# THUwangcy/ReChorus

Hardware: AMD Instinct MI355X
Metric: ranked (1+K)-tuples/sec (higher is better)
Workload: dtype f32; 1 GPU; BPRMF fit step: emb_size=64, num_neg=99, 10000001-item / 1000001-user tables, Zipf(1.0) users+positives, uniform negatives, B=65536 tuples/GPU/step, optimizer=SGD (row-wise, l2=0), int64 ids, fp32; batch_per_gpu=65536, num_neg=99, emb_size=64, n_items=10000001, optimizer=SGD, parallelism=single GPU

## Files before the change

include/rechorus_hip.h:

```cpp
#ifndef RECHORUS_HIP_H
#define RECHORUS_HIP_H

#include <stddef.h>
#include <stdint.h>

#ifdef __cplusplus
extern "C" {
#endif

typedef void* rc_stream_t;

enum rc_status {
  RC_OK = 0,
  RC_ERR_INVALID_ARG = -1,
  RC_ERR_WORKSPACE = -2,
  RC_ERR_HIP = -3,
  RC_ERR_UNSUPPORTED = -4
};

enum rc_opt {
  RC_OPT_SGD = 0,
  RC_OPT_ADAM = 1,
  RC_OPT_ADAGRAD = 2,
  RC_OPT_ADADELTA = 3
// ... 339 lines not shown
size_t rc_bucket_bitmap_bytes(int64_t range_a);
int rc_bucket_multi_bitmap(const int64_t* ids_a, int64_t n_a, int64_t range_a, uint32_t* bitmap, void* ws,
                           size_t ws_bytes, rc_stream_t stream);

size_t rc_plan_update_workspace_bytes(int64_t n_occ, int d);
int rc_plan_update(float* W, float* m, float* v, int d, const rc_plan_row* rows, const uint32_t* n_rows,
                   const uint32_t* occ, int64_t n_occ, const float* coef, const float* src, const int64_t* src_index,
                   int div, const float* src2, int64_t n_split, const rc_opt_hyper* h, void* ws, size_t ws_bytes,
                   rc_stream_t stream);

int rc_plan_update_pair(float* W_a, float* m_a, float* v_a, float* W_b, float* m_b, float* v_b, int d,
                        const rc_plan_row* rows, const uint32_t* n_rows, const uint32_t* occ, int64_t n_occ,
                        const float* src_a, const float* src_b, int64_t src_ld, int64_t occ_base, const rc_opt_hyper* h,
                        uint32_t* counters, void* ws, size_t ws_bytes, rc_stream_t stream);

int rc_plan_row_sums(float* out, int d, const rc_plan_row* rows, const uint32_t* n_rows, const uint32_t* occ,
                     int64_t n_occ, const float* coef, const float* src, const int64_t* src_index, int div,
                     const float* src2, int64_t n_split, void* ws, size_t ws_bytes, rc_stream_t stream);

int rc_plan_distinct(const rc_plan_row* rows, const uint32_t* n_rows, const uint32_t* occ, int64_t occ_base,
                     int64_t n_list, int64_t* uniq, int64_t* inverse, rc_stream_t stream);

size_t rc_bprmf_step_workspace_bytes(int B, int C, int d);

int rc_bprmf_step_pipeline(int mode);

int rc_bprmf_train_step(float* U, float* I, float* mU, float* vU, float* mI, float* vI,
                        const int64_t* uid, const int64_t* iid, int B, int C, int d,
                        int64_t n_users, int64_t n_items, const rc_opt_hyper* h,
                        float inv_b, float* loss_out, float* pred, void* ws,
                        size_t ws_bytes, rc_stream_t stream, float* phase_ms);

typedef struct rc_step_ticket {
  uint64_t generation;
  uint64_t ws;
  int32_t slot;
  int32_t device;
  int32_t B, C, d;
  int32_t flavour;
  int64_t n_users, n_items;
  uint64_t reserved[2];
} rc_step_ticket;

int rc_bprmf_train_step_ahead(float* U, float* I, float* mU, float* vU, float* mI, float* vI,
                              const int64_t* uid, const int64_t* iid, uint64_t generation,
                              const int64_t* next_uid, const int64_t* next_iid, uint64_t next_generation,
// ... 259 lines not shown
```

rechorus_amd/_lib.py:

```python
import ctypes as C
import os

_PKG = os.path.dirname(os.path.abspath(__file__))
LIB_PATH = os.environ.get("RC_LIB_PATH") or os.path.join(_PKG, "librechorus_hip.so")

RC_OK = 0
RC_OPT_SGD, RC_OPT_ADAM, RC_OPT_ADAGRAD, RC_OPT_ADADELTA = 0, 1, 2, 3
RC_SEG_SKIP_SINGLETONS = 1
OPT_BY_NAME = {"SGD": RC_OPT_SGD, "Adam": RC_OPT_ADAM, "Adagrad": RC_OPT_ADAGRAD, "Adadelta": RC_OPT_ADADELTA}


class RechorusHipMissing(ImportError):
    pass


class RechorusHipError(RuntimeError):
    def __init__(self, fn, code, text):
        super().__init__(f"{fn} failed (rc_status {code}): {text}")
        self.code = code


class OptHyper(C.Structure):
    _fields_ = [
        ("opt", C.c_int),
# ... 164 lines not shown
    "rc_neumf_head_fwd_bwd": (_i, [_p, _p, _i64, _p, _p, _i64, _p, _p, _p, _p, _p, _i, _i, _i, _i, _f, _p, _p, _p, _p, _i64, _p, _p, _i64,
                                   _p, _p, _p, _p, _sz, _p]),
    "rc_bench_mix": (_i, [_p, _i, _p, _i64, _f, _i, _p, C.POINTER(C.c_float), _p]),
    "rc_bench_mfma": (_i, [_i, _p, C.POINTER(C.c_float), _p]),
    "rc_linear_fwd": (_i, [_p, _p, _p, _i64, _i, _i, _i, _f, _p, C.c_uint32, _p, _p, _sz, _p]),
    "rc_linear_fwd_workspace_bytes": (_sz, [_i64, _i, _i]),
    "rc_linear_bwd_workspace_bytes": (_sz, [_i64, _i, _i]),
    "rc_linear_bwd": (_i, [_p, _p, _p, _p, _i64, _i, _i, _f, _i, _f, _p, _p, _p, _p, _sz, _p]),
    "rc_tower_tail_supported": (_i, [_i64, _i, _i]),
    "rc_tower_tail_workspace_bytes": (_sz, [_i64, _i, _i]),
    "rc_tower_tail_fwd": (_i, [_p, _p, _p, _p, _p, _i64, _i, _i, _f, _p, C.c_uint32, _p, _p, _p]),
    "rc_tower_tail_bwd": (_i, [_p, _p, _p, _p, _p, _i64, _i, _i, _f, _i, _f, _p, _p, _p, _p, _p, _p, _sz, _p]),
    "rc_bucket_plan_supported": (_i, [_i64, _i64, _i64, _i64]),
    "rc_bucket_plan_workspace_bytes": (_sz, [_i64, _i64]),
    "rc_bucket_plan_flags_bytes": (_sz, [_i64]),
    "rc_bucket_plan_status_ptr": (_p, [_p, _i64, _i64]),
    "rc_bucket_plan": (_i, [_p, _i64, _i64, _p, _i64, _i64, _i, _p, _p, _p, _p, _p, _p, _p, _sz, _p]),
    "rc_plan_update_workspace_bytes": (_sz, [_i64, _i]),
    "rc_plan_update": (_i, [_p, _p, _p, _i, _p, _p, _p, _i64, _p, _p, _p, _i, _p, _i64, _hp, _p, _sz, _p]),
    "rc_plan_update_pair": (_i, [_p, _p, _p, _p, _p, _p, _i, _p, _p, _p, _i64, _p, _p, _i64, _i64, _hp, _p, _p, _sz, _p]),
    "rc_plan_row_sums": (_i, [_p, _i, _p, _p, _p, _i64, _p, _p, _p, _i, _p, _i64, _p, _sz, _p]),
    "rc_plan_distinct": (_i, [_p, _p, _p, _i64, _i64, _p, _p, _p]),
    "rc_bprmf_step_workspace_bytes": (_sz, [_i, _i, _i]),
    "rc_bprmf_step_pipeline": (_i, [_i]),
    "rc_bprmf_train_step": (_i, [_p, _p, _p, _p, _p, _p, _p, _p, _i, _i, _i, _i64, _i64, _hp, _f,
                                 _p, _p, _p, _sz, _p, C.POINTER(C.c_float)]),
    "rc_bprmf_step_ahead_reset": (_i, [_tp, _p]),
    "rc_bprmf_train_step_ahead": (_i, [_p, _p, _p, _p, _p, _p, _p, _p, _u64, _p, _p, _u64, _tp, _i, _i, _i, _i64, _i64, _hp, _f,
                                       _p, _p, _p, _sz, _p, C.POINTER(C.c_float)]),
    "rc_bucket_bitmap_bytes": (_sz, [_i64]),
    "rc_bucket_multi_bitmap": (_i, [_p, _i64, _i64, _p, _p, _sz, _p]),
    "rc_lgcn_check_shape": (_i, [_i, _i, _i64, _i64]),
    "rc_lgcn_propagate_fwd": (_i, [_gp, _p, _p, _i, _i, _p, _p, _p, _p, _p]),
    "rc_lgcn_propagate_bwd": (_i, [_gp, _p, _p, _i, _i, _p, _p, _p, _p, _p, _p]),
    "rc_directau_check_shape": (_i, [_i, _i64]),
    "rc_directau_workspace_bytes": (_sz, [_i, _i64]),
    "rc_directau_fwd": (_i, [_p, _p, _p, _p, _i64, _i, _f, _i, _p, _sz, _p, _p, _p]),
    "rc_directau_bwd": (_i, [_p, _i64, _i, _f, _f, _f, _p, _sz, _p, _p, _p]),
    "rc_buir_check_shape": (_i, [_i, _i64]),
    "rc_buir_workspace_bytes": (_sz, [_i, _i64]),
    "rc_buir_fwd": (_i, [_p] * 8 + [_i64, _i, _p, _sz, _p, _p, _p]),
    "rc_buir_bwd": (_i, [_p] * 9 + [_i64, _i, _p, _sz, _p, _p, _p, _p, _p]),
    "rc_buir_query": (_i, [_p, _p, _p, _p, _i64, _i, _p, _p, _p]),
    "rc_buir_scores": (_i, [_p, _p, _p, _p, _i64, _i64, _i, _p, _p]),
    "rc_buir_ema": (_i, [_p, _p, _i64, _p, _p, _i64, _dbl, _p]),
    "rc_comirec_check_shape": (_i, [_i, _i, _i, _i]),
# ... 107 lines not shown
```

rechorus_amd/csrc/bprmf_fused.hip:

```cpp
#include "bprmf_step.hpp"
#include "fused_body.hpp"
#include "small_plan.hpp"

namespace rc {

template <int D, int GS, int CPL, int MODE>
__global__ __launch_bounds__(kBlock, (fused_min_waves<CPL, MODE>())) void bprmf_fwd_bwd_kernel(
    const float* __restrict__ U, const float* I,
    const int64_t* __restrict__ uid, const int64_t* __restrict__ iid, int B, int C,
    float inv_b, float* __restrict__ pred, float* __restrict__ loss_vec,
    float* __restrict__ gpred, float* __restrict__ ugrad, FusedUpd upd) {
  bprmf_fwd_bwd_body<D, GS, CPL, MODE, kBlock>(U, I, uid, iid, B, C, inv_b, pred, loss_vec, gpred, ugrad, upd,
                                               (int64_t)blockIdx.x, nullptr);
}

template <int D, int GS, int CPL>
__global__ __launch_bounds__(kSmallThreads) void small_front_kernel(
    const float* __restrict__ U, const float* I, const int64_t* __restrict__ uid, const int64_t* __restrict__ iid,
    int B, int C, float inv_b, float* __restrict__ pred, float* __restrict__ loss_vec, float* __restrict__ gpred,
    float* __restrict__ ugrad, float* __restrict__ ub, SmallPlanArgs plan) {
  extern __shared__ __attribute__((aligned(16))) unsigned char small_smem[];
  if (blockIdx.x < (unsigned)kSmallPlanWgs) {
    small_plan_block(plan, blockIdx.x, small_smem);
    return;
  }
  FusedUpd none;
  none.I = nullptr; none.M = nullptr; none.V = nullptr; none.single = nullptr;
  bprmf_fwd_bwd_body<D, GS, CPL, MODE_NONE, kSmallThreads>(U, I, uid, iid, B, C, inv_b, pred, loss_vec, gpred, ugrad, none,
                                                           (int64_t)blockIdx.x - kSmallPlanWgs, ub);
}

constexpr int kGenericMaxC = 4096;
constexpr int kGenericMaxDChunks = 8;

__global__ __launch_bounds__(kBlock) void bprmf_fwd_bwd_generic_kernel(
    const float* __restrict__ U, const float* __restrict__ I,
    const int64_t* __restrict__ uid, const int64_t* __restrict__ iid, int B, int C, int d,
    float inv_b, float* __restrict__ pred, float* __restrict__ loss_vec,
    float* __restrict__ gpred, float* __restrict__ ugrad) {
  extern __shared__ float smem[];
  const int lane = threadIdx.x & 63;
  const int wib = threadIdx.x >> 6;
  const int64_t t_raw = (int64_t)blockIdx.x * (kBlock / 64) + wib;
  const bool tv = t_raw < B;
  const int64_t t = tv ? t_raw : (int64_t)B - 1;
  float* sp = smem + (size_t)wib * C;
  const float* ur = U + uid[t] * d;
  const int64_t* ids = iid + t * C;
  for (int c = 0; c < C; ++c) {
    const float* ir = I + ids[c] * d;
// ... 61 lines not shown
  const float* U;
  const float* I;
  const int64_t* uid;
  const int64_t* iid;
  int B, C;
  float inv_b;
  float* pred;
  float* loss_vec;
  float* gpred;
  float* ugrad;
  int mode;
  const char* who;
  FusedUpd upd;
  hipStream_t s;
  const SmallPlanArgs* small;
  float* ub;
};

template <int D, int GS, int CPL>
static int launch_fused(const FusedCall& f) {
  constexpr int TPW = 64 / ((D / 4) * GS);
  constexpr int TPB = TPW * (kBlock / 64);
  const int blocks = (f.B + TPB - 1) / TPB;
  if (f.small) {
    constexpr int TPB_S = TPW * (kSmallThreads / 64);
    const int fblocks = (f.B + TPB_S - 1) / TPB_S;
    auto kern = small_front_kernel<D, GS, CPL>;
    static bool attr_done = false;
    if (!attr_done) {
      RC_HIP(hipFuncSetAttribute(reinterpret_cast<const void*>(kern), hipFuncAttributeMaxDynamicSharedMemorySize, (int)kSmallLdsBytes));
      attr_done = true;
    }
    hipLaunchKernelGGL(kern, dim3(kSmallPlanWgs + fblocks), dim3(kSmallThreads), kSmallLdsBytes, f.s, f.U, f.I, f.uid, f.iid,
                       f.B, f.C, f.inv_b, f.pred, f.loss_vec, f.gpred, f.ugrad, f.ub, *f.small);
    RC_LAUNCH_CHECK();
    return RC_OK;
  }
  return dispatch_or_fail<MODE_NONE, MODE_SGD, MODE_ADAM, MODE_ADAGRAD>(f.who, "update mode", f.mode, [&](auto M) -> int {
    hipLaunchKernelGGL((bprmf_fwd_bwd_kernel<D, GS, CPL, M()>), dim3(blocks), dim3(kBlock), 0, f.s, f.U, f.I, f.uid, f.iid, f.B, f.C,
                       f.inv_b, f.pred, f.loss_vec, f.gpred, f.ugrad, f.upd);
    RC_LAUNCH_CHECK();
    return RC_OK;
  });
}

template <int D>
// ... 53 lines not shown
  hipStream_t s = as_stream(stream);
  if (aligned16(U, I, ugrad) && register_path_ok(d, C)) {
    FusedCall f;
    memset(&f, 0, sizeof(f));
    f.U = U; f.I = I; f.uid = uid; f.iid = iid; f.B = B; f.C = C; f.inv_b = inv_b;
    f.pred = pred; f.loss_vec = loss_vec; f.gpred = gpred; f.ugrad = ugrad;
    f.mode = MODE_NONE; f.s = s; f.who = "rc_bprmf_fwd_bwd";
    bool handled = false;
    const int rc_ = run_fused(f, d, &handled);
    if (handled) return rc_;
  }
  if (C > kGenericMaxC || d > 64 * kGenericMaxDChunks)
    return fail(RC_ERR_UNSUPPORTED,
                "rc_bprmf_fwd_bwd: no kernel for C=%d d=%d (generic path: C<=%d, d<=%d)", C, d,
                kGenericMaxC, 64 * kGenericMaxDChunks);
  const int blocks = (B + (kBlock / 64) - 1) / (kBlock / 64);
  const size_t shmem = (size_t)(kBlock / 64) * C * sizeof(float);
  hipLaunchKernelGGL(bprmf_fwd_bwd_generic_kernel, dim3(blocks), dim3(kBlock), shmem, s, U, I,
                     uid, iid, B, C, d, inv_b, pred, loss_vec, gpred, ugrad);
  RC_LAUNCH_CHECK();
  return RC_OK;
}

extern "C" int rc_bprmf_fwd_bwd_update(const float* U, float* I, float* mI, float* vI, const int64_t* uid,
                                       const int64_t* iid, const uint8_t* single, const uint32_t* multi, int B, int C, int d,
                                       float inv_b, const rc_opt_hyper* h, float* pred, float* loss_vec, float* gpred, float* ugrad,
                                       rc_stream_t stream) {
  static const char* who = "rc_bprmf_fwd_bwd_update";
  if (B == 0) return RC_OK;
  RC_REQUIRE((single != nullptr) != (multi != nullptr), "%s: exactly one of single / multi must be given", who);
  RC_REQUIRE(U && I && uid && iid && h && loss_vec && gpred && ugrad, "%s: null pointer", who);
  RC_REQUIRE(B > 0 && C >= 2 && d >= 1, "%s: bad shape B=%d C=%d d=%d", who, B, C, d);
  if (!register_path_ok(d, C))
    return fail(RC_ERR_UNSUPPORTED,
                "%s: no register-resident kernel for d=%d C=%d "
                "(check rc_bprmf_fused_supported; use rc_bprmf_fwd_bwd + rc_segmented_update)", who, d, C);
  FusedCall f;
  memset(&f, 0, sizeof(f));
  RC_TRY(fill_opt_scalars(who, h, &f.upd.o));
  f.mode = mode_of(h);
  RC_TRY(opt_state_check(who, f.mode, mI != nullptr, vI != nullptr));
  RC_REQUIRE(aligned16(U, I, ugrad, mI, vI), "%s: tables must be 16-byte aligned", who);
  f.U = U; f.I = I; f.uid = uid; f.iid = iid; f.B = B; f.C = C; f.inv_b = inv_b;
  f.pred = pred; f.loss_vec = loss_vec; f.gpred = gpred; f.ugrad = ugrad;
  f.upd.I = I; f.upd.M = mI; f.upd.V = vI; f.upd.single = single; f.upd.multi = multi;
  f.s = as_stream(stream); f.who = who;
  bool handled = false;
  const int rc_ = run_fused(f, d, &handled);
  if (!handled) return fail(RC_ERR_UNSUPPORTED, "%s: dispatch failed", who);
  return rc_;
}

namespace rc {
int small_front_launch(const BprmfStep& st, float* ub, const SmallPlanArgs& plan) {
  const int d = st.d, C = st.C;
  RC_REQUIRE(aligned16(st.U, st.I, st.ugrad, ub) && register_path_ok(d, C),
             "small-batch step: unsupported shape or alignment (d=%d C=%d)", d, C);
  FusedCall f;
  memset(&f, 0, sizeof(f));
  f.U = st.U; f.I = st.I; f.uid = st.uid; f.iid = st.iid; f.B = st.B; f.C = C; f.inv_b = st.inv_b;
  f.pred = st.pred; f.loss_vec = st.loss_vec; f.gpred = st.gpred; f.ugrad = st.ugrad;
  f.mode = MODE_NONE; f.s = st.s; f.small = &plan; f.ub = ub; f.who = "rc_bprmf_train_step";
  bool handled = false;
  const int rc_ = run_fused(f, d, &handled);
  if (!handled) return fail(RC_ERR_UNSUPPORTED, "small-batch step: dispatch failed (d=%d C=%d)", d, C);
  return rc_;
}
}
```

rechorus_amd/csrc/bprmf_step.hpp:

```cpp
#pragma once
#include "common.hpp"
#include "opt_math.hpp"
#include "plan.hpp"

namespace rc {

struct SmallPlanArgs;

struct BprmfStep {
  float *U, *I;
  float *mU, *vU, *mI, *vI;
  const int64_t* uid;
  const int64_t* iid;
  int B, C, d;
  int64_t n_users, n_items;
  const rc_opt_hyper* h;
  OptScalars o;
  int mode;
  float inv_b;
  float* loss_out;
  float* pred;
  float *gpred, *ugrad, *loss_vec;
  hipStream_t s;
  int64_t n_i() const { return (int64_t)B * C; }
};

bool small_step_supported(int64_t n_i, int64_t B, int64_t n_items, int64_t n_users, int d);
size_t small_step_extra_bytes(int64_t n, int64_t B, int d);
int small_step_launch(const BprmfStep& st, void* extra, hipEvent_t* ev_mid);
int small_front_launch(const BprmfStep& st, float* ub, const SmallPlanArgs& plan);

int plan_bprmf_step_updates(const BprmfStep& st, const rc_plan_row* rows_i, const uint32_t* n_rows_i, const rc_plan_row* rows_u,
                            const uint32_t* n_rows_u, const uint32_t* occ, uint32_t* counters, const PlanLongWs& lw,
                            const PlanMedList& med, hipEvent_t* ev_items_done);

}
```

rechorus_amd/csrc/common.hpp:

```cpp
#pragma once
#include <cstdarg>
#include <cstdint>
#include <cstdio>
#include <cstring>
#include <cmath>
#include <type_traits>

#include <hip/hip_runtime.h>

#include "../../include/rechorus_hip.h"

namespace rc {

char* last_error_buf();

inline int fail(int code, const char* fmt, ...) {
  va_list ap;
  va_start(ap, fmt);
  vsnprintf(last_error_buf(), 512, fmt, ap);
  va_end(ap);
  return code;
}

#define RC_REQUIRE(cond, ...)                                   \
// ... 33 lines not shown

template <int... Vs, class F>
inline int dispatch_or_fail(const char* who, const char* what, int v, F&& f) {
  int rc = RC_OK;
  if (dispatch_int<Vs...>(v, &rc, f)) return rc;
  return fail(RC_ERR_UNSUPPORTED, "%s: %s %d has no kernel", who, what, v);
}

struct Carver {
  char* base;
  size_t off = 0;
  explicit Carver(void* p) : base(reinterpret_cast<char*>(p)) {}
  template <typename T>
  T* take(size_t count) {
    T* p = reinterpret_cast<T*>(base + off);
    off += align_up(count * sizeof(T), 256);
    return p;
  }
};

constexpr int kWave = 64;
constexpr int kBlock = 256;
constexpr int kMaxGridX = 1 << 30;

int device_cus();

#if defined(__HIPCC__)

template <int CTRL>
__device__ __forceinline__ float dpp_mov(float x) {
  int xi = __float_as_int(x);
  int r = __builtin_amdgcn_update_dpp(xi, xi, CTRL, 0xF, 0xF, false);
  return __int_as_float(r);
}

template <int NT, bool STAGED>
__device__ __forceinline__ float fixed_order_partial(const float* __restrict__ x, int64_t n, int tid) {
  float acc = 0.f;
  int64_t done = 0;
  if (reinterpret_cast<uintptr_t>(x) % 16 == 0) {
    const int64_t n4 = n / 4;
    const float4* x4 = reinterpret_cast<const float4*>(x);
    if (!STAGED || n4 <= (int64_t)4 * NT) {
#pragma unroll 8
      for (int64_t i = tid; i < n4; i += NT) {
        const float4 v = x4[i];
// ... 73 lines not shown
```

rechorus_amd/csrc/fused_body.hpp:

```cpp
#pragma once
#include "bpr_math.hpp"
#include "common.hpp"
#include "opt_math.hpp"

namespace rc {

struct FusedUpd {
  float* I;
  float* M;
  float* V;
  const uint8_t* single;
  const uint32_t* multi;
  OptScalars o;
};

template <int S>
__device__ __forceinline__ float tuple_allreduce_sum(float x) {
  x = row_allreduce_sum<(S < 16 ? S : 16)>(x);
  if (S >= 32) x += __shfl_xor(x, 16, 64);
  if (S >= 64) x += __shfl_xor(x, 32, 64);
  return x;
}
template <int S>
__device__ __forceinline__ float tuple_allreduce_max(float x) {
  if (S >= 2) x = fmaxf(x, dpp_mov<0xB1>(x));
  if (S >= 4) x = fmaxf(x, dpp_mov<0x4E>(x));
  if (S >= 8) x = fmaxf(x, dpp_mov<0x141>(x));
  if (S >= 16) x = fmaxf(x, dpp_mov<0x140>(x));
  if (S >= 32) x = fmaxf(x, __shfl_xor(x, 16, 64));
  if (S >= 64) x = fmaxf(x, __shfl_xor(x, 32, 64));
  return x;
}

template <int CPL_, int MODE_>
constexpr int fused_min_waves() {
  return (MODE_ == MODE_ADAM || MODE_ == MODE_ADAGRAD) ? (CPL_ >= 20 ? 2 : 3) : (CPL_ >= 26 ? 2 : (CPL_ >= 20 ? 3 : 4));
}
template <int D, int GS, int CPL>
struct FusedGeom {
  static constexpr int LPR = D / 4;
  static constexpr int S = LPR * GS;
  static_assert(S <= 64 && (64 % S) == 0, "tuple must fit a wave");
  static constexpr int TPW = 64 / S;
  static constexpr int SLOTS = GS * CPL;
  static constexpr int NPL = (SLOTS + S - 1) / S;
  static constexpr bool COAL = S == 64 && SLOTS <= 128;
  static constexpr int ID_SLOTS = COAL ? SLOTS : 1;
};

struct TupleIds {
  int64_t u;
  int64_t ia, ib;
};

template <int D, int GS, int CPL>
__device__ __forceinline__ TupleIds fused_load_ids(const int64_t* __restrict__ uid, const int64_t* __restrict__ iid, int64_t t,
                                                   int C, int lane) {
  using G = FusedGeom<D, GS, CPL>;
  TupleIds k;
  k.u = uid[t];
  k.ia = k.ib = 0;
  if (G::COAL) {
    const int64_t* ids = iid + t * C;
    const int c0 = lane, c1 = lane + 64;
    k.ia = ids[c0 < C ? c0 : 0];
    if (G::SLOTS > 64) k.ib = ids[c1 < C ? c1 : 0];
  }
  return k;
}

// ... 155 lines not shown
    if (cc[k] < 0) g = 0.f;
    if (s < SLOTS) strip[s] = g;
    if (tv && cc[k] >= 0) {
      gpred[t * C + cc[k]] = g;
      if (pred != nullptr) pred[t * C + cc[k]] = pc[k];
    }
  }
  __builtin_amdgcn_fence(__ATOMIC_RELEASE, "wavefront");
  __builtin_amdgcn_wave_barrier();
  __builtin_amdgcn_fence(__ATOMIC_ACQUIRE, "wavefront");

  float4 acc = make_float4(0.f, 0.f, 0.f, 0.f);
  float gs[CPL];
#pragma unroll
  for (int j = 0; j < CPL; ++j) {
    const float g = strip[grp * CPL + j];
    acc.x = fmaf(g, r[j].x, acc.x);
    acc.y = fmaf(g, r[j].y, acc.y);
    acc.z = fmaf(g, r[j].z, acc.z);
    acc.w = fmaf(g, r[j].w, acc.w);
    if (MODE == MODE_ADAM || MODE == MODE_ADAGRAD) gs[j] = g;
  }
  if (MODE == MODE_SGD) {
#pragma unroll
    for (int j = 0; j < CPL; ++j) {
      if (smask & (1u << j)) {
        const int64_t id = ids[j * GS + grp];
        const float g = strip[grp * CPL + j];
        const float4 gi = make_float4(g * u4.x, g * u4.y, g * u4.z, g * u4.w);
        opt_row4_group<MODE, LPR>(upd.o, upd.I, upd.M, upd.V, (size_t)id * LPR + l, r[j], gi);
      }
    }
  }
  acc.x = groups_allreduce_sum<LPR, S>(acc.x);
  acc.y = groups_allreduce_sum<LPR, S>(acc.y);
  acc.z = groups_allreduce_sum<LPR, S>(acc.z);
  acc.w = groups_allreduce_sum<LPR, S>(acc.w);
  if (tv && grp == 0) reinterpret_cast<float4*>(ugrad + t * D)[l] = acc;

  if (MODE == MODE_ADAM || MODE == MODE_ADAGRAD) {
    constexpr int GRP = 5;
#pragma unroll
    for (int j0 = 0; j0 < CPL; j0 += GRP) {
      float4 mm[GRP], vv[GRP];
      size_t idx[GRP];
#pragma unroll
      for (int q = 0; q < GRP; ++q) {
        const int j = j0 + q;
        mm[q] = vv[q] = make_float4(0.f, 0.f, 0.f, 0.f);
        idx[q] = 0;
        if (j < CPL && ((smask >> j) & 1u)) {
          idx[q] = (size_t)ids[j * GS + grp] * LPR + l;
          mm[q] = load_stream4(reinterpret_cast<const float4*>(upd.M) + idx[q]);
// ... 48 lines not shown
```

rechorus_amd/csrc/plan.hpp:

```cpp
#pragma once
#include "common.hpp"
#include "opt_math.hpp"

namespace rc {

constexpr int kPlanTile = 8192;
constexpr int kPlanThreads = 512;
constexpr int kPlanWaves = kPlanThreads / 64;
constexpr int kPlanRounds = kPlanTile / kPlanThreads;
constexpr int kPlanMaxBuckets = 4096;
constexpr int kPlanMaxShift = 13;
constexpr int kPlanMinShift = 8;
constexpr int kPlanLongSeg = 32;
constexpr int kPlanChunk = 256;
constexpr int kPlanIdxOcc = 4;
constexpr int kPlanBodyOcc = 2;

struct PlanGeom {
  int ok;
  int shift;
  uint32_t nb_a, nb_b, nb;
  uint32_t base_b;
  uint32_t tiles;
  int bucket_bits;
// ... 58 lines not shown
  int emit_long;
  PlanMedList med;
  int bitmap_in_bucket;
  PlanLongWs lw;
};
int plan_launch(const PlanArgs& a, hipStream_t s, hipEvent_t* ev_after_scatter);
int plan_launch_front(const PlanArgs& a, bool bitmap, hipStream_t s);
constexpr size_t kPlanBitmapWords = (size_t)kPlanMaxBuckets << (kPlanMaxShift - 5);
int plan_launch_back(const PlanArgs& a, hipStream_t s);
int plan_prepare();

struct PlanTable { float* W; float* M; float* V; };

struct PlanGrad {
  const float* coef;
  const float* src;
  const int64_t* src_index;
  int div;
  const float* src2;
  uint32_t n_split;
  const float* src2b;
  int pair;
  uint32_t pair_ld4;
};

}
```

rechorus_amd/csrc/plan_update.hip:

```cpp
#include "bprmf_step.hpp"
#include "plan.hpp"

namespace rc {

constexpr bool LPR_OK(int D) { return D / 4 <= 64 && 64 % (D / 4) == 0; }

struct PlanSide {
  PlanTable t;
  PlanTable tb;
  PlanGrad g;
  const rc_plan_row* rows;
  const uint32_t* n_rows;
};

struct PlanUpdArgs {
  PlanSide side[2];
  const uint32_t* occ;
  uint32_t* counters;
  PlanLongWs lw;
  OptScalars o;
  const float* loss_vec;
  int64_t loss_n;
  float loss_scale;
  float* loss_out;
// ... 103 lines not shown
#pragma unroll
    for (int h = 0; h < H; ++h) {
      if (g0 + h >= nr) break;
      if (!act[h]) {
        if (plan_long) plan_long_row<LPR>(a, e[h], side, l);
        continue;
      }
      if (e[h].n > 1) padd4(acc[h], s1[h]);
      if (!MED)
        for (uint32_t k = kPlanBodyOcc; k < e[h].n; ++k) padd4(acc[h], plan_grad4<D>(sd.g, a.occ, e[h].start + k, l));
      opt_row4_group<MODE, LPR>(a.o, tab[h].W, tab[h].M, tab[h].V, idx4[h], w[h], acc[h]);
    }
  }
}

template <int D, int MODE, bool MED = false>
__device__ __forceinline__ void plan_rows_indexed_body(const PlanUpdArgs& a, int side, bool plan_long, uint32_t first_block,
                                                       uint32_t n_blocks) {
  constexpr int LPR = D / 4;
  constexpr int GPW = 64 / LPR;
  constexpr int H = 2;
  constexpr uint32_t kIdxOcc = kPlanIdxOcc;
  constexpr uint32_t kMaxOcc = MED ? kPlanIdxOcc : kPlanLongSeg;
  const PlanSide& sd = a.side[side];
  const PlanGrad& gr = sd.g;
  const int lane = threadIdx.x & 63;
  const int l = lane % LPR, grp = lane / LPR;
  const uint32_t nr = *sd.n_rows;
  const uint32_t wave = (blockIdx.x - first_block) * (kBlock / 64) + (threadIdx.x >> 6);
  const uint32_t n_waves = n_blocks * (kBlock / 64);
  const float4* src4 = reinterpret_cast<const float4*>(gr.src);
  for (uint32_t base = wave * 64u; base < nr; base += n_waves * 64u) {
    const uint32_t gi = base + lane;
    rc_plan_row e;
    e.row = 0; e.start = 0; e.n = 0; e.reserved = 0;
    if (gi < nr) e = sd.rows[gi];
    const bool shortrow = e.n >= 1 && e.n <= kMaxOcc;
    uint32_t o0 = 0, o1 = 0, o2 = 0, o3 = 0;
    if (shortrow) {
      o0 = a.occ[e.start];
      if (e.n > 1) o1 = a.occ[e.start + 1];
      if (e.n > 2) o2 = a.occ[e.start + 2];
      if (e.n > 3) o3 = a.occ[e.start + 3];
    }
    float c0 = 1.0f, c1 = 1.0f, c2 = 1.0f, c3 = 1.0f;
    typedef int64_t src_row_t;
    src_row_t s0 = 0, s1 = 0, s2 = 0, s3 = 0;
    if (shortrow) {
      auto resolve = [&](uint32_t o, float& c, src_row_t& sr) {
        int64_t t = (gr.div == 1) ? (int64_t)o : (int64_t)(o / (uint32_t)gr.div);
        if (gr.src_index) t = gr.src_index[t];
        sr = (src_row_t)t;
        if (gr.coef) c = gr.coef[o];
      };
      resolve(o0, c0, s0);
      if (e.n > 1) resolve(o1, c1, s1);
      if (e.n > 2) resolve(o2, c2, s2);
      if (e.n > 3) resolve(o3, c3, s3);
    }
    for (int r0 = 0; r0 < 64; r0 += GPW * H) {
      if (base + (uint32_t)r0 >= nr) break;
      rc_plan_row eh[H];
      float ch0[H], ch1[H], ch2[H], ch3[H];
      src_row_t sh0[H], sh1[H], sh2[H], sh3[H];
      auto shfl64 = [](int64_t x, int sl) {
        return (int64_t)(((uint64_t)(uint32_t)__shfl((int)(uint32_t)(x >> 32), sl, 64) << 32) | (uint32_t)__shfl((int)(uint32_t)x, sl, 64));
      };
      bool on[H];
#pragma unroll
      for (int h = 0; h < H; ++h) {
        const int sl = r0 + h * GPW + grp;
        eh[h].row = __shfl(e.row, sl, 64);
        eh[h].start = __shfl(e.start, sl, 64);
        eh[h].n = __shfl(e.n, sl, 64);
        eh[h].reserved = 0;
        ch0[h] = __shfl(c0, sl, 64);
        ch1[h] = __shfl(c1, sl, 64);
        ch2[h] = __shfl(c2, sl, 64);
        ch3[h] = __shfl(c3, sl, 64);
        sh0[h] = shfl64(s0, sl);
        sh1[h] = shfl64(s1, sl);
        sh2[h] = shfl64(s2, sl);
        sh3[h] = shfl64(s3, sl);
        on[h] = eh[h].n >= 1 && eh[h].n <= kMaxOcc;
      }
      float4 w[H], m[H], v[H], u0[H], u1[H], u2[H], u3[H];
      size_t idx4[H];
#pragma unroll
      for (int h = 0; h < H; ++h) {
        idx4[h] = (size_t)eh[h].row * LPR + l;
        m[h] = v[h] = make_float4(0.f, 0.f, 0.f, 0.f);
        if (on[h]) {
          w[h] = load_stream4(reinterpret_cast<const float4*>(sd.t.W) + idx4[h]);
          if (mode_has_m(MODE)) m[h] = load_stream4(reinterpret_cast<const float4*>(sd.t.M) + idx4[h]);
          if (mode_has_v(MODE)) v[h] = load_stream4(reinterpret_cast<const float4*>(sd.t.V) + idx4[h]);
          u0[h] = src4[(size_t)sh0[h] * LPR + l];
          if (eh[h].n > 1) u1[h] = src4[(size_t)sh1[h] * LPR + l];
          if (eh[h].n > 2) u2[h] = src4[(size_t)sh2[h] * LPR + l];
          if (eh[h].n > 3) u3[h] = src4[(size_t)sh3[h] * LPR + l];
        }
      }
#pragma unroll
      for (int h = 0; h < H; ++h) {
        if (!on[h]) {
          if (plan_long && eh[h].n > (uint32_t)kPlanLongSeg) plan_long_row<LPR>(a, eh[h], side, l);
          continue;
        }
// ... 276 lines not shown
template <int D, int MODE>
static int launch_step_updates(const PlanUpdArgs& a_in, int64_t n_occ, hipStream_t s, hipEvent_t* ev_items_done) {
  constexpr uint32_t GPB = kBlock / (D / 4);
  PlanUpdArgs a = a_in;
  const uint32_t cus = (uint32_t)device_cus();
  const uint32_t blocks_main = cus * 32;
  const uint32_t med_max = (uint32_t)(n_occ / (kPlanBodyOcc + 1));
  a.blocks_med = med_max / GPB + 1 < cus ? med_max / GPB + 1 : cus;
  const uint32_t blocks_chunk = n_occ > kPlanLongSeg ? 512 : 0;
  hipLaunchKernelGGL((plan_rows_kernel<D, MODE, true>), dim3(a.blocks_med + blocks_chunk + blocks_main), dim3(kBlock), 0, s, a,
                     blocks_main, 0, 0, blocks_chunk);
  RC_LAUNCH_CHECK();
  if (ev_items_done) RC_HIP(hipEventRecord(*ev_items_done, s));
  const uint32_t blocks_rows = cus * 2;
  const uint32_t blocks_long = n_occ > kPlanLongSeg ? 256 : 0;
  hipLaunchKernelGGL((plan_final_kernel<D, MODE, true>), dim3(a.blocks_med + blocks_long + blocks_rows + 1), dim3(kBlock), 0, s, a,
                     blocks_rows, blocks_long, 1);
  RC_LAUNCH_CHECK();
  return RC_OK;
}

int plan_bprmf_step_updates(const BprmfStep& st, const rc_plan_row* rows_i, const uint32_t* n_rows_i, const rc_plan_row* rows_u,
                            const uint32_t* n_rows_u, const uint32_t* occ, uint32_t* counters, const PlanLongWs& lw,
                            const PlanMedList& med, hipEvent_t* ev_items_done) {
  const int64_t n_i = st.n_i();
  const int d = st.d;
  hipStream_t s = st.s;
  PlanUpdArgs a;
  memset(&a, 0, sizeof(a));
  a.long_planned = 1;
  a.med = med;
  a.chunk = kPlanChunk;
  a.o = st.o;
  a.side[0].t = PlanTable{st.I, st.mI, st.vI};
  a.side[0].g = PlanGrad{st.gpred, st.U, st.uid, st.C, nullptr, 0xFFFFFFFFu, nullptr, 0};
  a.side[0].rows = rows_i;
  a.side[0].n_rows = n_rows_i;
  a.side[1].t = PlanTable{st.U, st.mU, st.vU};
  a.side[1].g = PlanGrad{nullptr, nullptr, nullptr, 1, st.ugrad, (uint32_t)n_i, nullptr, 0};
  a.side[1].rows = rows_u;
  a.side[1].n_rows = n_rows_u;
  a.occ = occ;
  a.counters = counters;
  a.lw = lw;
  a.loss_vec = st.loss_vec;
  a.loss_n = st.B;
  a.loss_scale = st.inv_b;
  a.loss_out = st.loss_out;
  return dispatch_or_fail<MODE_SGD, MODE_ADAM, MODE_ADAGRAD>("rc_bprmf_train_step", "update mode", st.mode, [&](auto M) {
    constexpr int MODE = M;
    int rc = RC_OK;
    if (dispatch_int<16, 32, 64, 128>(d, &rc, [&](auto D) { return launch_step_updates<D(), MODE>(a, n_i + st.B, s, ev_items_done); }))
      return rc;
    return fail(RC_ERR_UNSUPPORTED, "plan update: d=%d (16/32/64/128)", d);
  });
}

}
// ... 140 lines not shown
```

rechorus_amd/csrc/train_step.hip:

```cpp
#include <mutex>

#include "bprmf_step.hpp"

namespace {
struct StepSide {
  hipStream_t stream = nullptr;
  hipEvent_t fork = nullptr, join = nullptr, fork2 = nullptr, front_done = nullptr;
  bool tried = false, ok = false;
};
constexpr int kMaxDevices = 64;
StepSide* step_side(int* device_out = nullptr) {
  static StepSide sides[kMaxDevices];
  static std::mutex mu;
  int dev = 0;
  if (hipGetDevice(&dev) != hipSuccess || dev < 0 || dev >= kMaxDevices) return nullptr;
  if (device_out) *device_out = dev;
  std::lock_guard<std::mutex> lock(mu);
  StepSide& x = sides[dev];
  if (!x.tried) {
    x.tried = true;
    x.ok = hipStreamCreateWithFlags(&x.stream, hipStreamNonBlocking) == hipSuccess &&
           hipEventCreateWithFlags(&x.fork, hipEventDisableTiming) == hipSuccess &&
           hipEventCreateWithFlags(&x.join, hipEventDisableTiming) == hipSuccess &&
           hipEventCreateWithFlags(&x.fork2, hipEventDisableTiming) == hipSuccess &&
// ... 2 lines not shown
  return x.ok ? &x : nullptr;
}
}

using namespace rc;

namespace {
struct PlanSlot {
  PlanWs plan;
  rc_plan_row* rows_i;
  rc_plan_row* rows_u;
  uint32_t* occ;
  uint32_t* bitmap;
  PlanLongWs plan_long;
};
struct StepWs {
  uint32_t* keys_i;
  uint32_t* perm_i;
  uint32_t* keys_u;
  uint32_t* perm_u;
  float* gpred;
  float* ugrad;
  float* loss_vec;
  uint8_t* single;
  uint32_t* heads_i;
  uint32_t* n_heads_i;
  void* sort_ws;
  size_t sort_ws_bytes;
  void* seg_ws;
  size_t seg_ws_bytes;
  PlanSlot slot[2];
  void* small_extra;
  size_t total;
};

StepWs carve_step_ws(void* base, int B, int C, int d) {
  const size_t n_i = (size_t)B * C;
  Carver cv(base);
  StepWs w;
  w.keys_i = cv.take<uint32_t>(n_i + (size_t)B);
  w.perm_i = cv.take<uint32_t>(n_i + (size_t)B);
  w.keys_u = w.keys_i + n_i;
  w.perm_u = w.perm_i + n_i;
  w.gpred = cv.take<float>(n_i);
  w.ugrad = cv.take<float>((size_t)B * d);
  w.loss_vec = cv.take<float>((size_t)B);
  const size_t plan_off = cv.off;
  w.single = cv.take<uint8_t>(n_i);
  w.heads_i = cv.take<uint32_t>(n_i);
  w.n_heads_i = cv.take<uint32_t>(1);
  w.sort_ws_bytes = rc_sort_workspace_bytes((int64_t)n_i + B);
  w.sort_ws = cv.take<char>(w.sort_ws_bytes);
  w.seg_ws_bytes = rc_segmented_workspace_bytes((int64_t)n_i, d);
  w.seg_ws = cv.take<char>(w.seg_ws_bytes);
  Carver pv(base);
  pv.off = plan_off;
  for (int k = 0; k < 2; ++k) {
    const PlanWs pw = carve_plan_ws(base ? reinterpret_cast<char*>(base) + pv.off : nullptr, (int64_t)n_i + B);
    w.slot[k].plan = pw;
    pv.off += align_up(pw.total, 256);
    w.slot[k].rows_i = pv.take<rc_plan_row>(n_i);
    w.slot[k].rows_u = pv.take<rc_plan_row>((size_t)B);
    w.slot[k].occ = pv.take<uint32_t>(n_i + (size_t)B);
    w.slot[k].bitmap = pv.take<uint32_t>(kPlanBitmapWords);
    const PlanLongWs lw = carve_plan_long_ws(base ? reinterpret_cast<char*>(base) + pv.off : nullptr, (int64_t)n_i + B, d);
    w.slot[k].plan_long = lw;
    pv.off += align_up(lw.total, 256);
  }
  w.total = cv.off > pv.off ? cv.off : pv.off;
// ... 25 lines not shown
  pa.lw = sl.plan_long;
  pa.med.end[0] = sl.rows_i + n_i; pa.med.cap[0] = (uint32_t)n_i; pa.med.over[0] = kPlanIdxOcc;
  pa.med.end[1] = sl.rows_u + B; pa.med.cap[1] = (uint32_t)B; pa.med.over[1] = kPlanBodyOcc;
  return pa;
}
}

static int& step_pipeline() {
  static int mode = 0;
  return mode;
}

extern "C" int rc_bprmf_step_pipeline(int mode) {
  const int prev = step_pipeline();
  if (mode >= 0 && mode <= 3) step_pipeline() = mode;
  return prev;
}

extern "C" size_t rc_bprmf_step_workspace_bytes(int B, int C, int d) {
  if (B < 1 || C < 1 || d < 1) return 0;
  return carve_step_ws(nullptr, B, C, d).total;
}

namespace {
class PhaseMarks {
 public:
  static constexpr int kMarks = 8;
  PhaseMarks() = default;
  PhaseMarks(const PhaseMarks&) = delete;
  PhaseMarks& operator=(const PhaseMarks&) = delete;
  ~PhaseMarks() {
    for (int i = 0; i < n_; ++i) (void)hipEventDestroy(ev_[i]);
  }
  int open(const float* phase_ms, hipStream_t s) {
    s_ = s;
    if (phase_ms != nullptr)
      for (; n_ < kMarks; ++n_) RC_HIP(hipEventCreate(&ev_[n_]));
    return RC_OK;
  }
  bool on() const { return n_ == kMarks; }
  int mark(int i) {
    if (on()) RC_HIP(hipEventRecord(ev_[i], s_));
    return RC_OK;
  }
  hipEvent_t* at(int i) { return on() ? &ev_[i] : nullptr; }
  int report(float* phase_ms) {
// ... 109 lines not shown
    RC_TRY(pm.mark(1));
    RC_HIP(hipEventRecord(side->fork, s));
    RC_HIP(hipStreamWaitEvent(side->stream, side->fork, 0));
    if (!fused_upd) RC_TRY(plan_launch_front(pa, false, side->stream));
    RC_TRY(plan_launch_back(pa, side->stream));
    RC_HIP(hipEventRecord(side->join, side->stream));
  } else {
    RC_TRY(plan_launch_front(pa, fused_upd, s));
    RC_TRY(pm.mark(1));
    RC_TRY(plan_launch_back(pa, s));
  }
  if (look_ahead) {
    PlanArgs pn = slot_plan_args(w, 1 - ah.slot, ah.next_uid, ah.next_iid, n_i, st.B, st.n_users, st.n_items, ch.geom, fused_upd);
    RC_HIP(hipEventRecord(side->fork2, s));
    RC_HIP(hipStreamWaitEvent(side->stream, side->fork2, 0));
    pn.bitmap_in_bucket = fused_upd ? 1 : 0;
    RC_TRY(plan_launch_front(pn, false, side->stream));
    RC_TRY(plan_launch_back(pn, side->stream));
    RC_HIP(hipEventRecord(side->front_done, side->stream));
    ticket_issue(ah, ws, 1 - ah.slot, st, ch.flavour);
  }
  RC_TRY(pm.mark(2));
  RC_TRY(pm.mark(3));
  if (fused_upd)
    RC_TRY(rc_bprmf_fwd_bwd_update(st.U, st.I, st.mI, st.vI, st.uid, st.iid, nullptr, w.slot[ah.slot].bitmap, st.B, st.C, st.d,
                                   st.inv_b, st.h, st.pred, st.loss_vec, st.gpred, st.ugrad, as_rc_stream(s)));
  else
    RC_TRY(rc_bprmf_fwd_bwd(st.U, st.I, st.uid, st.iid, st.B, st.C, st.d, st.inv_b, st.pred, st.loss_vec, st.gpred, st.ugrad,
                            as_rc_stream(s)));
  if (two_streams && !ah.hit) RC_HIP(hipStreamWaitEvent(s, side->join, 0));
  RC_TRY(pm.mark(4));
  RC_TRY(pm.mark(5));
  RC_TRY(plan_bprmf_step_updates(st, pa.rows_a, pa.n_rows_a, pa.rows_b, pa.n_rows_b, pa.occ, pa.w.counters, pa.lw, pa.med, pm.at(6)));
  return pm.mark(7);
}

int step_sort(const BprmfStep& st, const StepWs& w, bool fused_upd, PhaseMarks& pm) {
  const rc_stream_t stream = as_rc_stream(st.s);
  const int64_t n_i = st.n_i();
  RC_TRY(pm.mark(0));
  RC_TRY(rc_sort_ids(st.iid, n_i, st.uid, st.B, st.n_items, st.n_items + st.n_users, w.keys_i, w.perm_i, w.sort_ws, w.sort_ws_bytes,
                     stream));
  RC_TRY(pm.mark(1));
  if (fused_upd) RC_TRY(rc_segment_heads(w.keys_i, w.perm_i, n_i, 1, w.single, w.heads_i, w.n_heads_i, stream));
  RC_TRY(pm.mark(2));
  RC_TRY(pm.mark(3));
  if (fused_upd)
    RC_TRY(rc_bprmf_fwd_bwd_update(st.U, st.I, st.mI, st.vI, st.uid, st.iid, w.single, nullptr, st.B, st.C, st.d, st.inv_b, st.h,
                                   st.pred, st.loss_vec, st.gpred, st.ugrad, stream));
  else
    RC_TRY(rc_bprmf_fwd_bwd(st.U, st.I, st.uid, st.iid, st.B, st.C, st.d, st.inv_b, st.pred, st.loss_vec, st.gpred, st.ugrad, stream));
  RC_TRY(pm.mark(4));
  RC_TRY(rc_reduce_sum(st.loss_vec, st.B, st.inv_b, st.loss_out, stream));
  RC_TRY(pm.mark(5));
  RC_TRY(rc_segmented_update(st.I, st.mI, st.vI, st.d, w.keys_i, w.perm_i, n_i, st.gpred, st.U, st.uid, st.C, nullptr, n_i,
                             0, 0, st.h, nullptr, fused_upd ? w.heads_i : nullptr,
// ... 89 lines not shown
```

Baseline: 100.8 million tuples/s.

## Skip multi-occurrence SGD item updates whose summed step rounds away in fp32

The fused forward/backward kernel now also computes, for each non-single negative slot, a 2-bit headroom code. The code records whether |lr*g*u| is below a half- or quarter-ulp threshold of the current weight, and the codes are packed into per-tuple words stored in the reused sort-keys buffer. In SGD mode with l2=0, the medium-row plan update kernel reads these codes for rows with 2-4 occurrences. It drops rows whose combined update cannot change the stored fp32 weight, and compacts the remaining live rows with ballot/ffs instead of walking every slot. This aims to cut the gather/scatter traffic of many negative-item row updates, at the cost of extra per-slot arithmetic and code writes in the fused kernel. Exactness depends on the rounding thresholds being derived correctly.

```diff
diff --git a/include/rechorus_hip.h b/include/rechorus_hip.h
--- a/include/rechorus_hip.h
+++ b/include/rechorus_hip.h
@@ -385,6 +385,8 @@
                      int64_t n_list, int64_t* uniq, int64_t* inverse, rc_stream_t stream);
 
 size_t rc_bprmf_step_workspace_bytes(int B, int C, int d);
+
+size_t rc_bprmf_step_codes_offset(int B, int C, int d);
 
 int rc_bprmf_step_pipeline(int mode);
 
diff --git a/rechorus_amd/_lib.py b/rechorus_amd/_lib.py
--- a/rechorus_amd/_lib.py
+++ b/rechorus_amd/_lib.py
@@ -210,6 +210,7 @@
     "rc_plan_row_sums": (_i, [_p, _i, _p, _p, _p, _i64, _p, _p, _p, _i, _p, _i64, _p, _sz, _p]),
     "rc_plan_distinct": (_i, [_p, _p, _p, _i64, _i64, _p, _p, _p]),
     "rc_bprmf_step_workspace_bytes": (_sz, [_i, _i, _i]),
+    "rc_bprmf_step_codes_offset": (_sz, [_i, _i, _i]),
     "rc_bprmf_step_pipeline": (_i, [_i]),
     "rc_bprmf_train_step": (_i, [_p, _p, _p, _p, _p, _p, _p, _p, _i, _i, _i, _i64, _i64, _hp, _f,
                                  _p, _p, _p, _sz, _p, C.POINTER(C.c_float)]),
diff --git a/rechorus_amd/csrc/bprmf_fused.hip b/rechorus_amd/csrc/bprmf_fused.hip
--- a/rechorus_amd/csrc/bprmf_fused.hip
+++ b/rechorus_amd/csrc/bprmf_fused.hip
@@ -25,7 +25,7 @@
     return;
   }
   FusedUpd none;
-  none.I = nullptr; none.M = nullptr; none.V = nullptr; none.single = nullptr;
+  none.I = nullptr; none.M = nullptr; none.V = nullptr; none.single = nullptr; none.codes = nullptr;
   bprmf_fwd_bwd_body<D, GS, CPL, MODE_NONE, kSmallThreads>(U, I, uid, iid, B, C, inv_b, pred, loss_vec, gpred, ugrad, none,
                                                            (int64_t)blockIdx.x - kSmallPlanWgs, ub);
 }
@@ -133,6 +133,9 @@
   constexpr int TPW = 64 / ((D / 4) * GS);
   constexpr int TPB = TPW * (kBlock / 64);
   const int blocks = (f.B + TPB - 1) / TPB;
+  constexpr bool kCodes = FusedGeom<D, GS, CPL>::CODES;
+  if (f.upd.codes != nullptr && !(kCodes && f.mode == MODE_SGD))
+    return fail(RC_ERR_UNSUPPORTED, "%s: no headroom codes from the kernel for d=%d C=%d mode %d", f.who, D, f.C, f.mode);
   if (f.small) {
     constexpr int TPB_S = TPW * (kSmallThreads / 64);
     const int fblocks = (f.B + TPB_S - 1) / TPB_S;
@@ -232,11 +235,9 @@
   return RC_OK;
 }
 
-extern "C" int rc_bprmf_fwd_bwd_update(const float* U, float* I, float* mI, float* vI, const int64_t* uid,
-                                       const int64_t* iid, const uint8_t* single, const uint32_t* multi, int B, int C, int d,
-                                       float inv_b, const rc_opt_hyper* h, float* pred, float* loss_vec, float* gpred, float* ugrad,
-                                       rc_stream_t stream) {
-  static const char* who = "rc_bprmf_fwd_bwd_update";
+static int fwd_bwd_update(const char* who, const float* U, float* I, float* mI, float* vI, const int64_t* uid, const int64_t* iid,
+                          const uint8_t* single, const uint32_t* multi, int B, int C, int d, float inv_b, const rc_opt_hyper* h,
+                          float* pred, float* loss_vec, float* gpred, float* ugrad, uint32_t* codes, rc_stream_t stream) {
   if (B == 0) return RC_OK;
   RC_REQUIRE((single != nullptr) != (multi != nullptr), "%s: exactly one of single / multi must be given", who);
   RC_REQUIRE(U && I && uid && iid && h && loss_vec && gpred && ugrad, "%s: null pointer", who);
@@ -253,7 +254,7 @@
   RC_REQUIRE(aligned16(U, I, ugrad, mI, vI), "%s: tables must be 16-byte aligned", who);
   f.U = U; f.I = I; f.uid = uid; f.iid = iid; f.B = B; f.C = C; f.inv_b = inv_b;
   f.pred = pred; f.loss_vec = loss_vec; f.gpred = gpred; f.ugrad = ugrad;
-  f.upd.I = I; f.upd.M = mI; f.upd.V = vI; f.upd.single = single; f.upd.multi = multi;
+  f.upd.I = I; f.upd.M = mI; f.upd.V = vI; f.upd.single = single; f.upd.multi = multi; f.upd.codes = codes;
   f.s = as_stream(stream); f.who = who;
   bool handled = false;
   const int rc_ = run_fused(f, d, &handled);
@@ -261,7 +262,26 @@
   return rc_;
 }
 
+extern "C" int rc_bprmf_fwd_bwd_update(const float* U, float* I, float* mI, float* vI, const int64_t* uid,
+                                       const int64_t* iid, const uint8_t* single, const uint32_t* multi, int B, int C, int d,
+                                       float inv_b, const rc_opt_hyper* h, float* pred, float* loss_vec, float* gpred, float* ugrad,
+                                       rc_stream_t stream) {
+  return fwd_bwd_update("rc_bprmf_fwd_bwd_update", U, I, mI, vI, uid, iid, single, multi, B, C, d, inv_b, h, pred, loss_vec, gpred,
+                        ugrad, nullptr, stream);
+}
+
 namespace rc {
+bool fused_codes_supported(int d, int C) {
+  if (!register_path_ok(d, C) || (d != 32 && d != 64)) return false;
+  const int G = 256 / d;
+  return C > G / 2 && C <= 128;
+}
+
+int fused_step_launch(const BprmfStep& st, const uint32_t* multi, uint32_t* codes) {
+  return fwd_bwd_update("rc_bprmf_train_step", st.U, st.I, st.mI, st.vI, st.uid, st.iid, nullptr, multi, st.B, st.C, st.d, st.inv_b,
+                        st.h, st.pred, st.loss_vec, st.gpred, st.ugrad, codes, reinterpret_cast<rc_stream_t>(st.s));
+}
+
 int small_front_launch(const BprmfStep& st, float* ub, const SmallPlanArgs& plan) {
   const int d = st.d, C = st.C;
   RC_REQUIRE(aligned16(st.U, st.I, st.ugrad, ub) && register_path_ok(d, C),
diff --git a/rechorus_amd/csrc/bprmf_step.hpp b/rechorus_amd/csrc/bprmf_step.hpp
--- a/rechorus_amd/csrc/bprmf_step.hpp
+++ b/rechorus_amd/csrc/bprmf_step.hpp
@@ -30,8 +30,11 @@
 int small_step_launch(const BprmfStep& st, void* extra, hipEvent_t* ev_mid);
 int small_front_launch(const BprmfStep& st, float* ub, const SmallPlanArgs& plan);
 
+bool fused_codes_supported(int d, int C);
+int fused_step_launch(const BprmfStep& st, const uint32_t* multi, uint32_t* codes);
+
 int plan_bprmf_step_updates(const BprmfStep& st, const rc_plan_row* rows_i, const uint32_t* n_rows_i, const rc_plan_row* rows_u,
                             const uint32_t* n_rows_u, const uint32_t* occ, uint32_t* counters, const PlanLongWs& lw,
-                            const PlanMedList& med, hipEvent_t* ev_items_done);
+                            const PlanMedList& med, hipEvent_t* ev_items_done, const uint32_t* codes);
 
 }
diff --git a/rechorus_amd/csrc/common.hpp b/rechorus_amd/csrc/common.hpp
--- a/rechorus_amd/csrc/common.hpp
+++ b/rechorus_amd/csrc/common.hpp
@@ -79,6 +79,7 @@
 constexpr int kWave = 64;
 constexpr int kBlock = 256;
 constexpr int kMaxGridX = 1 << 30;
+constexpr int kCodeWords = 8;
 
 int device_cus();
 
diff --git a/rechorus_amd/csrc/fused_body.hpp b/rechorus_amd/csrc/fused_body.hpp
--- a/rechorus_amd/csrc/fused_body.hpp
+++ b/rechorus_amd/csrc/fused_body.hpp
@@ -12,7 +12,40 @@
   const uint8_t* single;
   const uint32_t* multi;
   OptScalars o;
+  uint32_t* codes;
 };
+
+constexpr float kCodeThr1 = 0.49951171875f - 0x1p-21f;
+constexpr float kCodeThr2 = 0.249755859375f - 0x1p-22f;
+
+__device__ __forceinline__ float code_inv_hs(float w, uint32_t& lo, uint32_t& hi) {
+  const uint32_t ef = (__float_as_uint(w) - 1u) & 0x7f800000u;
+  lo = ef < lo ? ef : lo;
+  hi = ef > hi ? ef : hi;
+  return __uint_as_float((278u << 23) - ef);
+}
+
+__device__ __forceinline__ float code_quot4(const float4& w, const float4& u, float p) {
+  uint32_t lo = 0xffffffffu, hi = 0u;
+  const float a = (p * fabsf(u.x)) * code_inv_hs(w.x, lo, hi);
+  const float b = (p * fabsf(u.y)) * code_inv_hs(w.y, lo, hi);
+  const float c = (p * fabsf(u.z)) * code_inv_hs(w.z, lo, hi);
+  const float d = (p * fabsf(u.w)) * code_inv_hs(w.w, lo, hi);
+  const bool ok = lo >= (64u << 23) && hi <= (253u << 23);
+  return ok ? fmaxf(fmaxf(a, b), fmaxf(c, d)) : INFINITY;
+}
+
+template <int LPR>
+__device__ __forceinline__ unsigned row_allreduce_and(unsigned x) {
+  auto dpp = [](unsigned v, auto ctrl) { return (unsigned)__builtin_amdgcn_update_dpp((int)v, (int)v, decltype(ctrl)::value, 0xF, 0xF, false); };
+  if (LPR >= 2) x &= dpp(x, std::integral_constant<int, 0xB1>{});
+  if (LPR >= 4) x &= dpp(x, std::integral_constant<int, 0x4E>{});
+  if (LPR >= 8) x &= dpp(x, std::integral_constant<int, 0x141>{});
+  if (LPR >= 16) x &= dpp(x, std::integral_constant<int, 0x140>{});
+  if (LPR >= 32) x &= (unsigned)__shfl_xor((int)x, 16, 64);
+  if (LPR >= 64) x &= (unsigned)__shfl_xor((int)x, 32, 64);
+  return x;
+}
 
 template <int S>
 __device__ __forceinline__ float tuple_allreduce_sum(float x) {
@@ -46,6 +79,7 @@
   static constexpr int NPL = (SLOTS + S - 1) / S;
   static constexpr bool COAL = S == 64 && SLOTS <= 128;
   static constexpr int ID_SLOTS = COAL ? SLOTS : 1;
+  static constexpr bool CODES = COAL && LPR >= kCodeWords && D <= 64;
 };
 
 struct TupleIds {
@@ -247,6 +281,11 @@
     if (MODE == MODE_ADAM || MODE == MODE_ADAGRAD) gs[j] = g;
   }
   if (MODE == MODE_SGD) {
+    const bool with_codes = G::CODES && upd.codes != nullptr;
+    const bool u_ok = fabsf(u4.x) < 0x1p100f && fabsf(u4.y) < 0x1p100f && fabsf(u4.z) < 0x1p100f && fabsf(u4.w) < 0x1p100f;
+    const float alr = u_ok ? fabsf(upd.o.neg_lr) : INFINITY;
+    const bool lr_zero = upd.o.neg_lr == 0.f;
+    unsigned lt1 = 0, lt2 = 0;
 #pragma unroll
     for (int j = 0; j < CPL; ++j) {
       if (smask & (1u << j)) {
@@ -254,6 +293,32 @@
         const float g = strip[grp * CPL + j];
         const float4 gi = make_float4(g * u4.x, g * u4.y, g * u4.z, g * u4.w);
         opt_row4_group<MODE, LPR>(upd.o, upd.I, upd.M, upd.V, (size_t)id * LPR + l, r[j], gi);
+      } else if (with_codes) {
+        const float g = strip[grp * CPL + j];
+        float p = fabsf(g) * alr;
+        if (!((p >= 0x1p-126f || g == 0.f || lr_zero) && fabsf(g) <= 0x1p20f)) p = INFINITY;
+        const float m = code_quot4(r[j], u4, p);
+        if (m < kCodeThr1) lt1 |= 1u << j;
+        if (m < kCodeThr2) lt2 |= 1u << j;
+      }
+    }
+    if constexpr (G::CODES) {
+      if (with_codes) {
+        lt1 = row_allreduce_and<LPR>(lt1);
+        lt2 = row_allreduce_and<LPR>(lt2);
+        const int nj = C > grp ? (C - grp + GS - 1) / GS : 0;
+        const unsigned multi = (nj >= 32 ? 0xffffffffu : (1u << nj) - 1u) & ~smask;
+        const uint64_t b0 = lt1 & ~lt2 & multi, b1 = lt2 & multi;
+        constexpr int JPW = 16 / GS;
+        uint32_t word = 0;
+#pragma unroll
+        for (int jj = 0; jj < JPW; ++jj) {
+          const int j = (l & (kCodeWords - 1)) * JPW + jj;
+          word |= (uint32_t)(((b0 >> j) & 1ull) | (((b1 >> j) & 1ull) << 1)) << (2 * (jj * GS + grp));
+        }
+#pragma unroll
+        for (int off = LPR; off < S; off <<= 1) word |= (uint32_t)__shfl_xor((int)word, off, 64);
+        if (tv && sub < kCodeWords) upd.codes[t * kCodeWords + sub] = word;
       }
     }
   }
diff --git a/rechorus_amd/csrc/plan.hpp b/rechorus_amd/csrc/plan.hpp
--- a/rechorus_amd/csrc/plan.hpp
+++ b/rechorus_amd/csrc/plan.hpp
@@ -104,6 +104,7 @@
   const float* src2b;
   int pair;
   uint32_t pair_ld4;
+  const uint32_t* codes;
 };
 
 }
diff --git a/rechorus_amd/csrc/plan_update.hip b/rechorus_amd/csrc/plan_update.hip
--- a/rechorus_amd/csrc/plan_update.hip
+++ b/rechorus_amd/csrc/plan_update.hip
@@ -149,6 +149,7 @@
   constexpr int H = 2;
   constexpr uint32_t kIdxOcc = kPlanIdxOcc;
   constexpr uint32_t kMaxOcc = MED ? kPlanIdxOcc : kPlanLongSeg;
+  constexpr bool SKIP = MED && MODE == MODE_SGD;
   const PlanSide& sd = a.side[side];
   const PlanGrad& gr = sd.g;
   const int lane = threadIdx.x & 63;
@@ -170,10 +171,22 @@
       if (e.n > 2) o2 = a.occ[e.start + 2];
       if (e.n > 3) o3 = a.occ[e.start + 3];
     }
+    bool live = shortrow;
+    if constexpr (SKIP) {
+      if (gr.codes != nullptr && e.n >= 2 && shortrow) {
+        auto code = [&](uint32_t o) {
+          const uint32_t t = o / (uint32_t)gr.div, c = o - t * (uint32_t)gr.div;
+          return (gr.codes[(size_t)t * kCodeWords + (c >> 4)] >> (2 * (c & 15u))) & 3u;
+        };
+        const uint32_t k0 = code(o0), k1 = code(o1), k2 = e.n > 2 ? code(o2) : 3u, k3 = e.n > 3 ? code(o3) : 3u;
+        const uint32_t k01 = k0 < k1 ? k0 : k1, k23 = k2 < k3 ? k2 : k3;
+        live = (k01 < k23 ? k01 : k23) < (e.n == 2 ? 1u : 2u);
+      }
+    }
     float c0 = 1.0f, c1 = 1.0f, c2 = 1.0f, c3 = 1.0f;
     typedef int64_t src_row_t;
     src_row_t s0 = 0, s1 = 0, s2 = 0, s3 = 0;
-    if (shortrow) {
+    if (SKIP ? live : shortrow) {
       auto resolve = [&](uint32_t o, float& c, src_row_t& sr) {
         int64_t t = (gr.div == 1) ? (int64_t)o : (int64_t)(o / (uint32_t)gr.div);
         if (gr.src_index) t = gr.src_index[t];
@@ -185,8 +198,20 @@
       if (e.n > 2) resolve(o2, c2, s2);
       if (e.n > 3) resolve(o3, c3, s3);
     }
+    uint64_t todo = SKIP ? (uint64_t)__ballot(live) : 0ull;
     for (int r0 = 0; r0 < 64; r0 += GPW * H) {
-      if (base + (uint32_t)r0 >= nr) break;
+      if (SKIP ? todo == 0ull : base + (uint32_t)r0 >= nr) break;
+      int pick[H];
+      if constexpr (SKIP) {
+#pragma unroll
+        for (int h = 0; h < H; ++h) pick[h] = -1;
+#pragma unroll
+        for (int q = 0; q < GPW * H; ++q) {
+          const int b = __ffsll((unsigned long long)todo) - 1;
+          todo &= todo - 1ull;
+          if (q % GPW == grp) pick[q / GPW] = b;
+        }
+      }
       rc_plan_row eh[H];
       float ch0[H], ch1[H], ch2[H], ch3[H];
       src_row_t sh0[H], sh1[H], sh2[H], sh3[H];
@@ -196,7 +221,7 @@
       bool on[H];
 #pragma unroll
       for (int h = 0; h < H; ++h) {
-        const int sl = r0 + h * GPW + grp;
+        const int sl = SKIP ? (pick[h] & 63) : r0 + h * GPW + grp;
         eh[h].row = __shfl(e.row, sl, 64);
         eh[h].start = __shfl(e.start, sl, 64);
         eh[h].n = __shfl(e.n, sl, 64);
@@ -209,7 +234,7 @@
         sh1[h] = shfl64(s1, sl);
         sh2[h] = shfl64(s2, sl);
         sh3[h] = shfl64(s3, sl);
-        on[h] = eh[h].n >= 1 && eh[h].n <= kMaxOcc;
+        on[h] = SKIP ? pick[h] >= 0 : (eh[h].n >= 1 && eh[h].n <= kMaxOcc);
       }
       float4 w[H], m[H], v[H], u0[H], u1[H], u2[H], u3[H];
       size_t idx4[H];
@@ -532,7 +557,7 @@
 
 int plan_bprmf_step_updates(const BprmfStep& st, const rc_plan_row* rows_i, const uint32_t* n_rows_i, const rc_plan_row* rows_u,
                             const uint32_t* n_rows_u, const uint32_t* occ, uint32_t* counters, const PlanLongWs& lw,
-                            const PlanMedList& med, hipEvent_t* ev_items_done) {
+                            const PlanMedList& med, hipEvent_t* ev_items_done, const uint32_t* codes) {
   const int64_t n_i = st.n_i();
   const int d = st.d;
   hipStream_t s = st.s;
@@ -544,6 +569,7 @@
   a.o = st.o;
   a.side[0].t = PlanTable{st.I, st.mI, st.vI};
   a.side[0].g = PlanGrad{st.gpred, st.U, st.uid, st.C, nullptr, 0xFFFFFFFFu, nullptr, 0};
+  a.side[0].g.codes = codes;
   a.side[0].rows = rows_i;
   a.side[0].n_rows = n_rows_i;
   a.side[1].t = PlanTable{st.U, st.mU, st.vU};
diff --git a/rechorus_amd/csrc/train_step.hip b/rechorus_amd/csrc/train_step.hip
--- a/rechorus_amd/csrc/train_step.hip
+++ b/rechorus_amd/csrc/train_step.hip
@@ -48,6 +48,8 @@
   float* gpred;
   float* ugrad;
   float* loss_vec;
+  uint32_t* codes;
+  size_t codes_off;
   uint8_t* single;
   uint32_t* heads_i;
   uint32_t* n_heads_i;
@@ -71,6 +73,9 @@
   w.gpred = cv.take<float>(n_i);
   w.ugrad = cv.take<float>((size_t)B * d);
   w.loss_vec = cv.take<float>((size_t)B);
+  const bool code_room = n_i + (size_t)B >= (size_t)B * kCodeWords;
+  w.codes = code_room ? w.keys_i : nullptr;
+  w.codes_off = code_room ? (size_t)(reinterpret_cast<char*>(w.keys_i) - cv.base) : ~(size_t)0;
   const size_t plan_off = cv.off;
   w.single = cv.take<uint8_t>(n_i);
   w.heads_i = cv.take<uint32_t>(n_i);
@@ -142,6 +147,11 @@
   return carve_step_ws(nullptr, B, C, d).total;
 }
 
+extern "C" size_t rc_bprmf_step_codes_offset(int B, int C, int d) {
+  if (B < 1 || C < 1 || d < 1) return ~(size_t)0;
+  return carve_step_ws(nullptr, B, C, d).codes_off;
+}
+
 namespace {
 class PhaseMarks {
  public:
@@ -297,16 +307,18 @@
   }
   RC_TRY(pm.mark(2));
   RC_TRY(pm.mark(3));
+  uint32_t* codes = nullptr;
+  if (fused_upd && st.mode == MODE_SGD && st.o.l2 == 0.0f && fabsf(st.o.neg_lr) <= 1048576.0f && fused_codes_supported(st.d, st.C))
+    codes = w.codes;
   if (fused_upd)
-    RC_TRY(rc_bprmf_fwd_bwd_update(st.U, st.I, st.mI, st.vI, st.uid, st.iid, nullptr, w.slot[ah.slot].bitmap, st.B, st.C, st.d,
-                                   st.inv_b, st.h, st.pred, st.loss_vec, st.gpred, st.ugrad, as_rc_stream(s)));
+    RC_TRY(fused_step_launch(st, w.slot[ah.slot].bitmap, codes));
   else
     RC_TRY(rc_bprmf_fwd_bwd(st.U, st.I, st.uid, st.iid, st.B, st.C, st.d, st.inv_b, st.pred, st.loss_vec, st.gpred, st.ugrad,
                             as_rc_stream(s)));
   if (two_streams && !ah.hit) RC_HIP(hipStreamWaitEvent(s, side->join, 0));
   RC_TRY(pm.mark(4));
   RC_TRY(pm.mark(5));
-  RC_TRY(plan_bprmf_step_updates(st, pa.rows_a, pa.n_rows_a, pa.rows_b, pa.n_rows_b, pa.occ, pa.w.counters, pa.lw, pa.med, pm.at(6)));
+  RC_TRY(plan_bprmf_step_updates(st, pa.rows_a, pa.n_rows_a, pa.rows_b, pa.n_rows_b, pa.occ, pa.w.counters, pa.lw, pa.med, pm.at(6), codes));
   return pm.mark(7);
 }
 
```

New measurement: 108.0 million tuples/s, median of 6. 1.07x the previous value.
